# zuston/TonY

Hardware: AMD Instinct MI355X
Metric: images/sec (whole node) Inception-v3 TF-PS (higher is better)
Workload: dtype bf16

## Files before the change

### tony_amd/models/inception_v3.py

```python
from __future__ import annotations

import os

import torch
from torch import nn

from ..ops.concat import Slot, assemble, concat_buffer
from ..ops.dropout import Dropout as TonyDropout
from ..ops.pool import avg_pool, avg_pool3x3_s1, global_avg_pool, max_pool
from ..ops import conv as conv_ops
from ..ops import streams, tape
from ..ops.fused import FusedHead
from ..ops.residual import GradJoin
from ..ops.linear import Linear
from ..ops.x3 import ConvBNActX3, LinearX3, split_act
from .layers import ConvBNAct, conv_bn_act_maxpool, init_weights


JOIN = os.environ.get("TONY_INCEPTION_JOIN", "1") != "0"


def _join(t: torch.Tensor, n: int) -> None:
    if JOIN and t.is_cuda and t.dtype in (torch.bfloat16, torch.float32) and torch.is_grad_enabled() \
            and t.requires_grad:
        t._tony_join = GradJoin(n)


def _x3_input(x: torch.Tensor) -> None:
    if x.is_cuda and x.dtype == torch.float32:
        split_act(x)

# ... 365 lines not shown
            stem = (self.stem, self.stem2)
            segs = [(self._stem_fwd, [p for m in stem for p in m.parameters()], [b for m in stem for b in m.buffers()])]
            for blk in (*self.mixed_5, self.mixed_6a, *self.mixed_6):
                segs.append((blk, list(blk.parameters()), list(blk.buffers())))
            tail = [(blk, list(blk.parameters()), list(blk.buffers())) for blk in self.mixed_7]
            segs = self._tape_segs = (segs, tail)
        return segs

    def forward(self, x):
        if (self.fused and self.training and x.is_cuda and tape.ENABLED and torch.is_grad_enabled()
                and x.shape[0] * 64 >= conv_ops.MIN_ROWS):
            head, tail = self._segments()
            for run, params, bufs in head:
                x = tape.segment(run, x, params, bufs)
            aux = self.aux(x) if self.aux is not None else None
            for run, params, bufs in tail:
                x = tape.segment(run, x, params, bufs)
        else:
            x = self._stem_fwd(x)
            x = self.mixed_6(self.mixed_6a(self.mixed_5(x)))
            aux = self.aux(x) if (self.aux is not None and self.training) else None
            x = self.mixed_7(x)
        if self.fused or self.x3:
            x = global_avg_pool(x)
        else:
            x = torch.flatten(nn.functional.adaptive_avg_pool2d(x, 1), 1)
        logits = self.fc(self.dropout(x))
        return (logits, aux) if aux is not None else logits


def inception_v3(num_classes=1000, aux_logits=True, fused=True, seed=0, precision: str = "bf16") -> InceptionV3:
    if precision not in ("bf16", "fp32"):
        raise ValueError(f"precision must be bf16 or fp32, not {precision!r}")
    return init_weights(InceptionV3(num_classes, aux_logits, fused=fused, x3=precision == "fp32"), seed)
```

### tony_amd/models/resnet.py

```python
from __future__ import annotations

import os

import torch
from torch import nn

from ..ops import conv as conv_ops
from ..ops.bn import BatchNormAct2d
from ..ops.linear import Linear
from ..ops.pool import global_avg_pool
from ..ops.residual import GradJoin, bn_add_relu, conv1x1_bn_add_relu
from .layers import ConvBNAct, conv_bn_act_maxpool, init_weights


JOIN = os.environ.get("TONY_RESNET_JOIN", "1") != "0"
DS_TONY = os.environ.get("TONY_RESNET_DS_TONY", "1") != "0"


class Bottleneck(nn.Module):
    expansion = 4

    def __init__(self, cin, width, stride=1, fused=True, eps=1e-5):
        super().__init__()
        cout = width * self.expansion
        self.fused = fused
        self.conv1 = ConvBNAct(cin, width, 1, fused=fused, eps=eps)
        self.conv2 = ConvBNAct(width, width, 3, stride=stride, padding=1, fused=fused, eps=eps)
        self.conv3 = nn.Conv2d(width, cout, 1, bias=False)
        self.bn3 = nn.BatchNorm2d(cout, eps=eps)
        self.downsample = None
        if stride != 1 or cin != cout:
            self.downsample = nn.Sequential(
                nn.Conv2d(cin, cout, 1, stride=stride, bias=False),
# ... 26 lines not shown


class ResNet(nn.Module):
    def __init__(self, layers=(3, 4, 6, 3), num_classes=1000, fused=True, eps=1e-5):
        super().__init__()
        self.fused = fused
        self.stem = ConvBNAct(3, 64, 7, stride=2, padding=3, fused=fused, eps=eps)
        blocks = []
        cin = 64
        for i, n in enumerate(layers):
            width = 64 * 2 ** i
            for j in range(n):
                blocks.append(Bottleneck(cin, width, stride=2 if (j == 0 and i > 0) else 1, fused=fused, eps=eps))
                cin = width * Bottleneck.expansion
        self.blocks = nn.Sequential(*blocks)
        self.fc = (Linear if fused else nn.Linear)(cin, num_classes)

    def forward(self, x):
        if self.fused:
            x = conv_bn_act_maxpool(self.stem, x, 3, 2, padding=1)
        else:
            x = torch.nn.functional.max_pool2d(self.stem(x), 3, 2, 1)
        x = self.blocks(x)
        x = global_avg_pool(x) if self.fused else x.mean((2, 3))
        return self.fc(x)


def resnet50(num_classes: int = 1000, fused: bool = True, seed: int = 0) -> ResNet:
    m = ResNet((3, 4, 6, 3), num_classes, fused=fused)
    init_weights(m, seed)
    for b in m.blocks:
        nn.init.zeros_(b.bn3.weight)
    return m
```

### tony_amd/ops/_lib.py

```python
from __future__ import annotations

import ctypes
import os
import threading
import weakref
from typing import Dict

import torch

_HERE = os.path.dirname(os.path.abspath(__file__))
SO_PATH = os.environ.get("TONY_KERNELS_SO") or os.path.join(_HERE, "_tony_kernels.so")

_lock = threading.Lock()
_lib = None

c_void_p = ctypes.c_void_p
c_int = ctypes.c_int
c_int64 = ctypes.c_int64
c_float = ctypes.c_float
c_int_p = ctypes.POINTER(ctypes.c_int)
c_void_pp = ctypes.POINTER(ctypes.c_void_p)
c_u8_p = ctypes.POINTER(ctypes.c_uint8)
c_u64_p = ctypes.POINTER(ctypes.c_uint64)

# ... 50 lines not shown
    "tony_sgd_step": [c_void_p, c_void_p, c_void_p, c_int, c_void_p, c_int64, c_void_p, c_void_p],
    "tony_adam_step": [c_void_p, c_void_p, c_void_p, c_void_p, c_int, c_void_p, c_int64, c_void_p, c_void_p],
    "tony_adagrad_step": [c_void_p, c_void_p, c_void_p, c_int, c_void_p, c_int64, c_void_p, c_void_p],
    "tony_rmsprop_step": [c_void_p, c_void_p, c_void_p, c_void_p, c_int, c_void_p, c_int64, c_void_p, c_void_p],
    "tony_grad_stats": [c_void_p, c_int, c_int64, c_void_p, c_void_p],
    "tony_grad_sumsq_blocks": [],
    "tony_grad_sumsq": [c_void_p, c_int, c_int64, c_void_p, c_void_p],
    "tony_clip_ctl": [c_void_p, c_int, c_void_p, c_void_p, c_void_p],
    "tony_optim_apply_x": [c_int, c_void_p, c_void_p, c_void_p, c_void_p, c_void_p, c_int, c_void_p, c_int64,
                           c_void_p, c_void_p, c_void_p, c_void_p],
    "tony_layerwise_item_floats": [],
    "tony_lars_norm": [c_void_p, c_void_p, c_int, c_void_p, c_int64, c_void_p, c_int, c_void_p, c_void_p, c_void_p],
    "tony_lamb_norm": [c_void_p, c_void_p, c_void_p, c_void_p, c_int, c_int64, c_void_p, c_int, c_void_p, c_void_p,
                       c_void_p, c_void_p, c_void_p],
    "tony_layerwise_fold": [c_void_p, c_void_p, c_void_p, c_int, c_void_p, c_void_p],
    "tony_layerwise_ratio": [c_int, c_void_p, c_void_p, c_int, c_void_p, c_void_p, c_void_p, c_void_p],
    "tony_lars_apply": [c_void_p, c_void_p, c_void_p, c_void_p, c_int, c_void_p, c_int64, c_void_p, c_int, c_void_p,
                        c_void_p, c_void_p, c_void_p, c_void_p],
    "tony_lamb_apply": [c_void_p, c_void_p, c_void_p, c_void_p, c_void_p, c_int64, c_void_p, c_int, c_void_p,
                        c_void_p, c_void_p, c_void_p, c_void_p],
    "tony_xent_fwd": [c_void_p, c_int, c_int64, c_int, c_int64, c_void_p, c_float, c_void_p, c_void_p, c_void_p],
    "tony_xent_bwd": [c_void_p, c_int, c_int64, c_int, c_int64, c_void_p, c_float, c_void_p, c_void_p, c_void_p,
                      c_int64, c_void_p],
    "tony_image_preprocess": [c_void_p, c_int, c_void_p, c_void_p, c_int, c_int, c_int, c_int, c_int, c_int, c_float,
                              c_float, c_float, c_float, c_float, c_float, c_void_p],
    "tony_image_colour_scratch_floats": [c_int, c_int, c_int],
    "tony_image_preprocess_colour": [c_void_p, c_int, c_void_p, c_void_p, c_int, c_void_p, c_int64, c_void_p, c_int,
                                     c_int, c_int, c_int, c_int, c_int, c_float, c_float, c_float, c_float, c_float,
                                     c_float, c_void_p],
    "tony_topk_count": [c_void_p, c_int, c_int64, c_int, c_int64, c_void_p, c_int, c_void_p, c_void_p],
    "tony_dropout_fwd": [c_void_p, c_void_p, c_void_p, c_int64, c_int, c_float, c_void_p, c_void_p],
    "tony_dropout_bwd": [c_void_p, c_void_p, c_void_p, c_int64, c_int, c_float, c_void_p],
    "tony_counter_bump": [c_void_p, c_void_p],
    "tony_gemm_bf16": [c_void_p, c_void_p, c_void_p, c_int64, c_int64, c_int64, c_int64, c_int64, c_int64,
                       c_int, c_void_p, c_int64, c_void_p],
    "tony_gemm_bf16_bnact": [c_void_p, c_void_p, c_void_p, c_int64, c_int64, c_int64, c_int64, c_int64, c_int64,
                             c_int, c_void_p, c_int64, c_void_p, c_void_p],
    "tony_gemm_tn_bf16": [c_void_p, c_void_p, c_void_p, c_int64, c_int64, c_int64, c_int64, c_int64, c_int64,
                          c_void_p, c_int64, c_void_p, c_int, c_void_p, c_void_p, c_int, c_void_p],
    "tony_splitk_reduce": [c_void_p, c_int, c_int64, c_void_p, c_int, c_int, c_int, c_void_p],
    "tony_splitk_workspace": [c_void_p, c_int64, c_void_p, c_int64],
    "tony_conv_fwd": [c_void_p, c_int, c_int, c_int, c_int, c_int64, c_void_p, c_int, c_int, c_int, c_int, c_int,
                      c_int, c_int, c_void_p, c_int, c_int, c_int64, c_int, c_void_p, c_int64, c_void_p],
    "tony_stem_fwd": [c_void_p, c_int, c_int, c_int, c_int, c_void_p, c_int, c_int, c_int, c_int, c_int, c_int,
                      c_int, c_void_p, c_int, c_int, c_int64, c_int, c_void_p, c_int64, c_int, c_void_p],
    "tony_stem_wgrad": [c_void_p, c_int64, c_void_p, c_int, c_int, c_int, c_int, c_int, c_int, c_int, c_int, c_int,
# ... 371 lines not shown
```

### tony_amd/ops/conv.py

```python
from __future__ import annotations

import ctypes
import os
import weakref
from typing import Callable, Dict, Tuple

import torch

from . import _lib, concat, streams, tape, tune, wt_cache
from .arena import zeros_f32
from .bn import HOST_MEMO, _accum_ok, _as_rows, _rows_view
from .gemm import occ_choices, splitk_combine, wgrad_cus, wgrad_tn

_BF16 = torch.bfloat16
AUTOTUNE = os.environ.get("TONY_CONV_AUTOTUNE", "1") != "0"
_CHOICE: Dict[Tuple, str] = {}


def _pair(v):
    if type(v) is tuple:
        return v
    return tuple(v) if isinstance(v, (tuple, list)) else (int(v), int(v))


STEM = os.environ.get("TONY_STEM", "1") != "0"
MIN_ROWS = int(os.environ.get("TONY_CONV_MIN_ROWS", "1"))


_SUP_CACHE: dict = {}


def supported(x: torch.Tensor, weight: torch.Tensor, stride=1, padding=0, dilation=1, groups=1,
# ... 296 lines not shown
    return x if _rows_view(x)[2] == x.shape[1] else x.contiguous(memory_format=torch.channels_last)


def _gemm_fwd(x, weight, stats=None):
    x = _dense_rows(x)
    n = x.shape[0]
    co = weight.shape[0]
    k = x[0].numel()
    _lib.check_stat_buffer(stats, co)
    wk = _krsc(weight).reshape(co, k)
    y = _cl_empty(n, co, 1, 1, x.device)
    vf = tune.gemm_flags(x, wk, y, n, co, k, k, stats is not None, tune.SMALL_GEMM_VARIANTS)
    rc = _lib.lib().tony_gemm_bf16(x.data_ptr(), wk.data_ptr(), y.data_ptr(), n, co, k, k, k, co,
                                   (1 if stats is not None else 0) | vf, _lib.ptr(stats),
                                   2 * co if stats is not None else 0, _lib.stream_ptr(x.device))
    _lib.check(rc, "tony_gemm_bf16 (whole-input conv)")
    return y


def _gemm_dgrad(dy, weight, x_shape):
    dy, (_, co, lddy) = _as_rows(dy)
    n, c, h, w = x_shape
    k = c * h * w
    wt = _krsc(weight).reshape(co, k).t().contiguous()
    dx = _cl_empty(n, c, h, w, dy.device)
    if lddy != co:
        dy = dy.contiguous(memory_format=torch.channels_last)
        lddy = co
    vf = tune.gemm_flags(dy, wt, dx, n, k, co, lddy, False, tune.SMALL_GEMM_VARIANTS)
    rc = _lib.lib().tony_gemm_bf16(dy.data_ptr(), wt.data_ptr(), dx.data_ptr(), n, k, co, lddy, co, k, vf, 0, 0,
                                   _lib.stream_ptr(dy.device))
    _lib.check(rc, "tony_gemm_bf16 (whole-input conv dgrad)")
    return dx


def _gemm_wgrad(dy, x, weight_shape, dst=None):
    dy, (_, co, lddy) = _as_rows(dy)
    x = _dense_rows(x)
    n = x.shape[0]
    k = x[0].numel()
    if n % 8 == 0 and (dst is None or dst.dtype in (torch.float32, _BF16)):
        dev = x.device
        dyt = torch.as_strided(dy, (co, n), (1, lddy)).contiguous()
        xt = x.permute(0, 2, 3, 1).reshape(n, k).t().contiguous()
        out = dst if dst is not None else torch.empty(co * k, dtype=torch.float32, device=dev)
        base = (8 if out.dtype == torch.float32 else 0) | (16 if dst is not None else 0)
        scratch = torch.empty(co * k, dtype=_BF16, device=dev)
# ... 412 lines not shown
```

### tony_amd/ops/csrc/loss.hip

```cpp
#include "common.h"

using namespace tony;

namespace {

constexpr int kThreads = 256;
constexpr int kPerThread = 16;

template <bool kBf16>
__device__ __forceinline__ float ld(const void* p, int64_t i) {
  if constexpr (kBf16) return bf2f(static_cast<const uint16_t*>(p)[i]);
  return static_cast<const float*>(p)[i];
}

__device__ __forceinline__ float block_reduce(float v, float* sh, bool is_max) {
  v = is_max ? wave_max(v) : wave_sum(v);
  const int lane = threadIdx.x & (kWave - 1), wid = threadIdx.x / kWave;
  __syncthreads();
  if (lane == 0) sh[wid] = v;
  __syncthreads();
  float r = sh[0];
#pragma unroll
  for (int k = 1; k < kThreads / kWave; ++k) r = is_max ? fmaxf(r, sh[k]) : r + sh[k];
  return r;
}

template <bool kBf16>
__global__ __launch_bounds__(kThreads) void xent_fwd_kernel(const void* __restrict__ logits, int64_t ld_,
                                                            int K, const int64_t* __restrict__ labels,
                                                            float smoothing, float* __restrict__ loss,
                                                            float* __restrict__ lse_out) {
  __shared__ float sh[kThreads / kWave];
  const int64_t row = blockIdx.x;
  const int64_t base = row * ld_;
  float v[kPerThread];
  float mx = -INFINITY;
#pragma unroll
  for (int j = 0; j < kPerThread; ++j) {
    const int k = threadIdx.x + j * kThreads;
    v[j] = k < K ? ld<kBf16>(logits, base + k) : -INFINITY;
    mx = fmaxf(mx, v[j]);
  }
  mx = block_reduce(mx, sh, true);
  float se = 0.f, sx = 0.f;
#pragma unroll
  for (int j = 0; j < kPerThread; ++j) {
    const int k = threadIdx.x + j * kThreads;
    if (k < K) {
      se += __expf(v[j] - mx);
      sx += v[j];
    }
  }
  se = block_reduce(se, sh, false);
  sx = block_reduce(sx, sh, false);
  if (threadIdx.x == 0) {
    const float lse = mx + __logf(se);
    const int64_t t = labels[row];
    const bool live = t >= 0 && t < K;
    const float xt = live ? ld<kBf16>(logits, base + t) : lse;
    float l = (1.f - smoothing) * (lse - xt);
    if (smoothing != 0.f) l += smoothing * (lse - sx / static_cast<float>(K));
    loss[row] = live ? l : 0.f;
    lse_out[row] = lse;
  }
}

template <bool kBf16>
__global__ __launch_bounds__(kThreads) void xent_bwd_kernel(const void* __restrict__ logits, int64_t ld_,
                                                            int K, const int64_t* __restrict__ labels,
                                                            float smoothing, const float* __restrict__ lse,
                                                            const float* __restrict__ gout,
                                                            void* __restrict__ dlogits, int64_t ldd) {
  const int64_t row = blockIdx.x;
  const float l = lse[row];
  const float go = gout[row];
  const int64_t t = labels[row];
  const bool live = t >= 0 && t < K;
  const float off = smoothing / static_cast<float>(K);
  for (int k = threadIdx.x; k < K; k += kThreads) {
    const float p = __expf(ld<kBf16>(logits, row * ld_ + k) - l);
    const float target = (k == t ? 1.f - smoothing : 0.f) + off;
    const float d = live ? (p - target) * go : 0.f;
    if constexpr (kBf16)
      static_cast<uint16_t*>(dlogits)[row * ldd + k] = f2bf(d);
    else
      static_cast<float*>(dlogits)[row * ldd + k] = d;
  }
}

}

TONY_API int tony_xent_fwd(const void* logits, int is_bf16, int64_t N, int K, int64_t ld_,
                           const int64_t* labels, float smoothing, float* loss, float* lse,
                           hipStream_t stream) {
  if (K <= 0 || K > kThreads * kPerThread) return -1;
  if (N <= 0) return 0;
  if (is_bf16)
    xent_fwd_kernel<true><<<N, kThreads, 0, stream>>>(logits, ld_, K, labels, smoothing, loss, lse);
  else
    xent_fwd_kernel<false><<<N, kThreads, 0, stream>>>(logits, ld_, K, labels, smoothing, loss, lse);
  TONY_LAUNCH_CHECK();
  return 0;
}

TONY_API int tony_xent_bwd(const void* logits, int is_bf16, int64_t N, int K, int64_t ld_,
                           const int64_t* labels, float smoothing, const float* lse, const float* gout,
                           void* dlogits, int64_t ldd, hipStream_t stream) {
  if (K <= 0) return -1;
  if (N <= 0) return 0;
  if (is_bf16)
    xent_bwd_kernel<true><<<N, kThreads, 0, stream>>>(logits, ld_, K, labels, smoothing, lse, gout, dlogits, ldd);
  else
    xent_bwd_kernel<false><<<N, kThreads, 0, stream>>>(logits, ld_, K, labels, smoothing, lse, gout, dlogits, ldd);
  TONY_LAUNCH_CHECK();
  return 0;
}
```

### tony_amd/ops/linear.py

```python
from __future__ import annotations

import os

import torch
from torch import nn

from . import _lib, tape, tune
from .gemm import wgrad_tn

_BF16 = torch.bfloat16
TUNE = os.environ.get("TONY_LINEAR_TUNE", "1") != "0"


def supported(x: torch.Tensor, weight: torch.Tensor) -> bool:
    return (x.is_cuda and x.dtype == _BF16 and weight.dtype == _BF16 and x.dim() == 2
            and weight.shape[1] % 8 == 0 and weight.shape[0] % 8 == 0 and x.shape[1] == weight.shape[1])


def _affine(bias: torch.Tensor | None, n: int, device) -> torch.Tensor:
    aff = torch.zeros(2 * n, dtype=torch.float32, device=device)
    aff[:n] = 1.0
    if bias is not None:
        aff[n:] = bias.float()
    return aff


class _LinearFn(torch.autograd.Function):
    @staticmethod
    def forward(ctx, x, weight, bias):
        L = _lib.lib()
        if x.stride(1) != 1 or x.data_ptr() % 16 or x.stride(0) % 8:
            x = x.contiguous()
        w = weight if weight.is_contiguous() else weight.contiguous()
        m, k = x.shape
        n = w.shape[0]
        y = torch.empty((m, n), dtype=x.dtype, device=x.device)
        aff = _affine(bias, n, x.device)
        vf = tune.gemm_flags(x, w, y, m, n, k, x.stride(0), False) if TUNE else 0
        rc = L.tony_gemm_bf16(x.data_ptr(), w.data_ptr(), y.data_ptr(), m, n, k, x.stride(0), k, n, 2 | vf,
                              aff.data_ptr(), 0, _lib.stream_ptr(x.device))
        _lib.check(rc, "tony_gemm_bf16 (linear)")
        ctx.save_for_backward(x, w)
        ctx.has_bias = bias is not None
        ctx.params = (weight, bias)
        return y

    @staticmethod
    def backward(ctx, dy):
        x, w = ctx.saved_tensors
        weight, bias = ctx.params
        L, dev = _lib.lib(), x.device
        st = _lib.stream_ptr(dev)
        if dy.stride(1) != 1 or dy.data_ptr() % 16 or dy.stride(0) % 8:
            dy = dy.contiguous()
        m, k = x.shape
        n = w.shape[0]
        dx = dw = db = None
        if ctx.needs_input_grad[0]:
            wt = w.t().contiguous()
            dx = torch.empty((m, k), dtype=x.dtype, device=dev)
            vf = tune.gemm_flags(dy, wt, dx, m, k, n, dy.stride(0), False) if TUNE else 0
            rc = L.tony_gemm_bf16(dy.data_ptr(), wt.data_ptr(), dx.data_ptr(), m, k, n, dy.stride(0), n, k, vf, 0, 0,
                                  st)
            _lib.check(rc, "tony_gemm_bf16 (linear dgrad)")
        if ctx.needs_input_grad[1]:
            gw = _lib.grad_slot(weight)
            if gw is not None and gw.is_contiguous():
                wgrad_tn(dy.data_ptr(), dy.stride(0), x.data_ptr(), x.stride(0), m, n, k, dev, dst=gw)
            else:
                dw = wgrad_tn(dy.data_ptr(), dy.stride(0), x.data_ptr(), x.stride(0), m, n, k, dev).to(weight.dtype)
        if ctx.has_bias and ctx.needs_input_grad[2]:
            db = dy.float().sum(0)
            gb = _lib.grad_slot(bias)
            if gb is not None:
                gb.add_(db.to(gb.dtype))
                db = None
            else:
                db = db.to(bias.dtype)
        _lib.report_inplace((weight, bias), (dw, db))
        return dx, dw, db


def linear(x: torch.Tensor, weight: torch.Tensor, bias: torch.Tensor | None = None) -> torch.Tensor:
    if supported(x, weight):
        return tape.apply(_LinearFn, x, weight, bias)
    return nn.functional.linear(x, weight, bias)


class Linear(nn.Linear):

    def forward(self, x):
        return linear(x, self.weight, self.bias)
```

### tony_amd/ops/loss.py

```python
from __future__ import annotations

import torch

from . import _lib


class _XentFn(torch.autograd.Function):
    @staticmethod
    def forward(ctx, logits, labels, smoothing):
        L = _lib.lib()
        if logits.stride(1) != 1:
            logits = logits.contiguous()
        labels = labels.contiguous().to(torch.int64)
        n, k = logits.shape
        is_bf16 = int(logits.dtype == torch.bfloat16)
        if not is_bf16 and logits.dtype != torch.float32:
            raise TypeError(f"cross_entropy kernel takes bf16/fp32 logits, got {logits.dtype}")
        loss = torch.empty(n, dtype=torch.float32, device=logits.device)
        lse = torch.empty(n, dtype=torch.float32, device=logits.device)
        rc = L.tony_xent_fwd(logits.data_ptr(), is_bf16, n, k, logits.stride(0), labels.data_ptr(), float(smoothing),
                             loss.data_ptr(), lse.data_ptr(), _lib.stream_ptr(logits.device))
        _lib.check(rc, "tony_xent_fwd")
        ctx.save_for_backward(logits, labels, lse)
        ctx.smoothing = smoothing
        return loss

    @staticmethod
    def backward(ctx, gout):
        L = _lib.lib()
        logits, labels, lse = ctx.saved_tensors
        n, k = logits.shape
        gout = gout.float().contiguous()
        if gout.numel() != n:
            gout = gout.expand(n).contiguous()
        d = torch.empty((n, k), dtype=logits.dtype, device=logits.device)
        rc = L.tony_xent_bwd(logits.data_ptr(), int(logits.dtype == torch.bfloat16), n, k, logits.stride(0),
                             labels.data_ptr(), float(ctx.smoothing), lse.data_ptr(), gout.data_ptr(), d.data_ptr(), k,
                             _lib.stream_ptr(logits.device))
        _lib.check(rc, "tony_xent_bwd")
        return d, None, None


def cross_entropy(logits: torch.Tensor, labels: torch.Tensor, label_smoothing: float = 0.0,
                  reduction: str = "mean") -> torch.Tensor:
    if logits.is_cuda:
        per_row = _XentFn.apply(logits, labels, label_smoothing)
    else:
        valid = (labels >= 0) & (labels < logits.shape[1])
        per_row = torch.nn.functional.cross_entropy(logits.float(), torch.where(valid, labels, -100),
                                                    reduction="none", ignore_index=-100,
                                                    label_smoothing=label_smoothing)
    if reduction == "mean":
        return per_row.mean()
    if reduction == "sum":
        return per_row.sum()
    return per_row
```

### tony_amd/ops/pool.py

```python
from __future__ import annotations

import torch

from . import _lib, concat, streams, tape
from .bn import _as_rows, _rows_view


def _nhwc_empty(n, c, h, w, like):
    return torch.empty((n, c, h, w), dtype=like.dtype, device=like.device, memory_format=torch.channels_last)


def _fn(name: str, t: torch.Tensor):
    return getattr(_lib.lib(), name + "_f32" if t.dtype == torch.float32 else name)


def _ok(x: torch.Tensor) -> bool:
    return x.is_cuda and x.dtype in (torch.bfloat16, torch.float32) and x.shape[1] % 8 == 0


def _dense_rows(t: torch.Tensor, shape) -> bool:
    if tuple(t.shape) != tuple(shape) or t.data_ptr() % 16:
        return False
    rv = _rows_view(t)
    return rv is not None and rv[2] == t.shape[1]


def _box3(src, n, c, h, w, ld_src):
# ... 98 lines not shown
        _lib.check(rc, "tony_avgpool_fwd")
        ctx.shape = (n, c, h, w, k, s)
        return y

    @staticmethod
    def backward(ctx, dy):
        n, c, h, w, k, s = ctx.shape
        dy, (_, _, lddy) = _as_rows(dy)
        dx = _nhwc_empty(n, c, h, w, dy)
        rc = _fn("tony_avgpool_bwd", dy)(dy.data_ptr(), dx.data_ptr(), n, h, w, c, k, s, lddy, c,
                                         _lib.stream_ptr(dy.device))
        _lib.check(rc, "tony_avgpool_bwd")
        return dx, None, None


def avg_pool(x: torch.Tensor, k: int, s: int) -> torch.Tensor:
    if _ok(x):
        return tape.apply(_AvgPoolFn, x, k, s)
    return torch.nn.functional.avg_pool2d(x, k, s)


def global_avg_pool(x: torch.Tensor) -> torch.Tensor:
    if x.shape[2] == x.shape[3]:
        return torch.flatten(avg_pool(x, x.shape[2], 1), 1)
    return torch.flatten(torch.nn.functional.adaptive_avg_pool2d(x, 1), 1)


def avg_pool3x3_s1(x: torch.Tensor, planes_only: bool = False) -> torch.Tensor:
    if _ok(x):
        planes_only = planes_only and x.dtype == torch.float32 and not tape.recording()
        _LAST_PLANES[0] = None
        y = tape.apply(_AvgPool3Fn, x, planes_only)
        planes = _LAST_PLANES[0]
        if planes is not None:
            _LAST_PLANES[0] = None
            y._tony_x3 = (y._version, planes, x.shape[1])
        return y
    return torch.nn.functional.avg_pool2d(x, 3, 1, 1, count_include_pad=True)


def max_pool(x: torch.Tensor, k: int = 3, s: int = 2, slot=None, padding: int = 0) -> torch.Tensor:
    if _ok(x) and 2 * padding <= k:
        return tape.apply(_MaxPoolFn, x, k, s, slot, padding)
    return torch.nn.functional.max_pool2d(x, k, s, padding)
```

### tony_amd/ops/wt_cache.py

```python
from __future__ import annotations

import struct
from typing import Dict, Optional

import torch

from . import _lib

_DESC = struct.Struct("<QQiiiiii")
_T = 64


def _crsk(weight: torch.Tensor) -> torch.Tensor:
    return weight.permute(1, 2, 3, 0).contiguous()


class TransposedWeights:
    def __init__(self, device):
        self.device = _norm(device)
        if _lib.lib().tony_transpose_desc_bytes() != _DESC.size:
            raise _lib.KernelError("transpose descriptor layout differs between Python and the kernels")
        self.entries: Dict[int, tuple] = {}
        self.enabled = False
        self.frozen = False
        self.desc: Optional[torch.Tensor] = None
        self.n_desc = 0
        self.total_tiles = 0

    def get(self, weight: torch.Tensor) -> Optional[torch.Tensor]:
        if not self.enabled or not isinstance(weight, torch.nn.Parameter) or weight.dim() != 4:
            return None
        e = self.entries.get(id(weight))
        if e is not None and e[0] is weight and e[2] == weight.data_ptr():
            return e[1]
        if self.frozen or torch.cuda.is_current_stream_capturing():
            return None
        co, ci, r, s = weight.shape
        if not weight.is_contiguous(memory_format=torch.channels_last) or weight.dtype != torch.bfloat16:
            return None
        buf = _crsk(weight)
        self.entries[id(weight)] = (weight, buf, weight.data_ptr())
        self._build()
        return buf

    def _build(self):
        parts, tiles = [], 0
        for w, buf, _ in self.entries.values():
            co, ci, r, s = w.shape
            tci, tco = (ci + _T - 1) // _T, (co + _T - 1) // _T
            parts.append(_DESC.pack(w.data_ptr(), buf.data_ptr(), co, r * s, ci, tci, tco, tiles))
            tiles += r * s * tci * tco
        raw = torch.frombuffer(bytearray(b"".join(parts)), dtype=torch.uint8)
        self.desc = raw.to(self.device)
        self.n_desc = len(parts)
        self.total_tiles = tiles

    def refresh(self) -> None:
        if not self.n_desc:
            return
        L = _lib.lib()
        rc = L.tony_transpose_batch(self.desc.data_ptr(), self.n_desc, self.total_tiles,
                                    _lib.stream_ptr(self.device))
        _lib.check(rc, "tony_transpose_batch")


_XDESC = struct.Struct("<QQQiiiiiiii")


class X3Weights:

    def __init__(self, device):
        self.device = _norm(device)
        if _lib.lib().tony_x3_desc_bytes() != _XDESC.size:
            raise _lib.KernelError("x3 weight descriptor layout differs between Python and the kernels")
# ... 63 lines not shown
        d = torch.device("cuda", torch.cuda.current_device())
    return d


def activate(cache: Optional[TransposedWeights], x3cache: Optional[X3Weights] = None) -> None:
    _ACTIVE[0] = cache
    _ACTIVE_X3[0] = x3cache


def x3_planes(weight: torch.Tensor) -> Optional[torch.Tensor]:
    c = _ACTIVE_X3[0]
    if c is not None and c.enabled and c.device == _norm(weight.device):
        return c.planes(weight)
    return None


def x3_planes_t(weight: torch.Tensor) -> Optional[torch.Tensor]:
    c = _ACTIVE_X3[0]
    if c is not None and c.enabled and c.device == _norm(weight.device):
        return c.planes_t(weight)
    return None


def transposed(weight: torch.Tensor) -> torch.Tensor:
    c = _ACTIVE[0]
    if c is not None and c.enabled and c.device == _norm(weight.device):
        t = c.get(weight)
        if t is not None:
            return t
    return _crsk(weight)
```

Before: 9752.

## Fuse classifier head: pool+dropout kernel, mean-xent, cached flat weight transposes, bias colsum

Adds HIP kernels that fuse global average pooling with dropout in forward and backward, and a cross-entropy kernel that folds the batch mean in-kernel using a last-block counter. The fc bias gradient is accumulated directly into the grad slot, and flat transposed weights for the fc and flat conv backward are cached in the batched transpose cache. The goal is to cut the many small launches and copies in the classifier head and loss. In exchange it adds a new dropout RNG path and atomic counter state that must work under graph capture.

```diff
diff --git a/tony_amd/models/inception_v3.py b/tony_amd/models/inception_v3.py
--- a/tony_amd/models/inception_v3.py
+++ b/tony_amd/models/inception_v3.py
@@ -7,6 +7,7 @@
 
 from ..ops.concat import Slot, assemble, concat_buffer
 from ..ops.dropout import Dropout as TonyDropout
+from ..ops.head import pool_dropout
 from ..ops.pool import avg_pool, avg_pool3x3_s1, global_avg_pool, max_pool
 from ..ops import conv as conv_ops
 from ..ops import streams, tape
@@ -418,10 +419,10 @@
             aux = self.aux(x) if (self.aux is not None and self.training) else None
             x = self.mixed_7(x)
         if self.fused or self.x3:
-            x = global_avg_pool(x)
-        else:
-            x = torch.flatten(nn.functional.adaptive_avg_pool2d(x, 1), 1)
-        logits = self.fc(self.dropout(x))
+            x = pool_dropout(x, self.dropout)
+        else:
+            x = self.dropout(torch.flatten(nn.functional.adaptive_avg_pool2d(x, 1), 1))
+        logits = self.fc(x)
         return (logits, aux) if aux is not None else logits
 
 
diff --git a/tony_amd/models/resnet.py b/tony_amd/models/resnet.py
--- a/tony_amd/models/resnet.py
+++ b/tony_amd/models/resnet.py
@@ -8,7 +8,7 @@
 from ..ops import conv as conv_ops
 from ..ops.bn import BatchNormAct2d
 from ..ops.linear import Linear
-from ..ops.pool import global_avg_pool
+from ..ops.head import pool_dropout
 from ..ops.residual import GradJoin, bn_add_relu, conv1x1_bn_add_relu
 from .layers import ConvBNAct, conv_bn_act_maxpool, init_weights
 
@@ -81,7 +81,7 @@
         else:
             x = torch.nn.functional.max_pool2d(self.stem(x), 3, 2, 1)
         x = self.blocks(x)
-        x = global_avg_pool(x) if self.fused else x.mean((2, 3))
+        x = pool_dropout(x) if self.fused else x.mean((2, 3))
         return self.fc(x)
 
 
diff --git a/tony_amd/ops/_lib.py b/tony_amd/ops/_lib.py
--- a/tony_amd/ops/_lib.py
+++ b/tony_amd/ops/_lib.py
@@ -96,6 +96,16 @@
     "tony_xent_fwd": [c_void_p, c_int, c_int64, c_int, c_int64, c_void_p, c_float, c_void_p, c_void_p, c_void_p],
     "tony_xent_bwd": [c_void_p, c_int, c_int64, c_int, c_int64, c_void_p, c_float, c_void_p, c_void_p, c_void_p,
                       c_int64, c_void_p],
+    "tony_xent_fwd_mean": [c_void_p, c_int, c_int64, c_int, c_int64, c_void_p, c_float, c_void_p, c_void_p, c_void_p,
+                           c_void_p, c_void_p],
+    "tony_xent_bwd_mean": [c_void_p, c_int, c_int64, c_int, c_int64, c_void_p, c_float, c_void_p, c_void_p, c_void_p,
+                           c_int64, c_void_p],
+    "tony_head_pool_dropout_fwd": [c_void_p, c_void_p, c_void_p, c_int, c_int, c_int, c_int64, c_int64, c_float,
+                                   c_void_p, c_void_p],
+    "tony_head_pool_dropout_bwd": [c_void_p, c_void_p, c_void_p, c_int, c_int, c_int, c_int64, c_int64, c_float,
+                                   c_void_p],
+    "tony_head_affine": [c_void_p, c_int, c_int, c_void_p, c_void_p],
+    "tony_colsum_accum": [c_void_p, c_int64, c_int, c_int, c_void_p, c_int, c_void_p],
     "tony_image_preprocess": [c_void_p, c_int, c_void_p, c_void_p, c_int, c_int, c_int, c_int, c_int, c_int, c_float,
                               c_float, c_float, c_float, c_float, c_float, c_void_p],
     "tony_image_colour_scratch_floats": [c_int, c_int, c_int],
diff --git a/tony_amd/ops/conv.py b/tony_amd/ops/conv.py
--- a/tony_amd/ops/conv.py
+++ b/tony_amd/ops/conv.py
@@ -7,7 +7,7 @@
 
 import torch
 
-from . import _lib, concat, streams, tape, tune, wt_cache
+from . import _lib, concat, head, streams, tape, tune, wt_cache
 from .arena import zeros_f32
 from .bn import HOST_MEMO, _accum_ok, _as_rows, _rows_view
 from .gemm import occ_choices, splitk_combine, wgrad_cus, wgrad_tn
@@ -350,7 +350,7 @@
     dy, (_, co, lddy) = _as_rows(dy)
     n, c, h, w = x_shape
     k = c * h * w
-    wt = _krsc(weight).reshape(co, k).t().contiguous()
+    wt = wt_cache.transposed_flat(weight) if head.FUSED else _krsc(weight).reshape(co, k).t().contiguous()
     dx = _cl_empty(n, c, h, w, dy.device)
     if lddy != co:
         dy = dy.contiguous(memory_format=torch.channels_last)
diff --git a/tony_amd/ops/csrc/head.hip b/tony_amd/ops/csrc/head.hip
--- /dev/null
+++ b/tony_amd/ops/csrc/head.hip
@@ -0,0 +1,193 @@
+#include "common.h"
+
+using namespace tony;
+
+namespace {
+
+constexpr int kLanes = 64;
+constexpr int kThreads = 256;
+
+__device__ __forceinline__ uint64_t mix64(uint64_t z) {
+  z += 0x9e3779b97f4a7c15ull;
+  z = (z ^ (z >> 30)) * 0xbf58476d1ce4e5b9ull;
+  z = (z ^ (z >> 27)) * 0x94d049bb133111ebull;
+  return z ^ (z >> 31);
+}
+
+__device__ __forceinline__ unsigned keep_bits(const int64_t* rng, int64_t g, uint32_t thr) {
+  const uint64_t key =
+      mix64(static_cast<uint64_t>(rng[0]) ^ mix64(static_cast<uint64_t>(rng[1]) + 0x632be59bd9b4e019ull));
+  const uint64_t h0 = mix64(key + 2 * static_cast<uint64_t>(g)), h1 = mix64(key + 2 * static_cast<uint64_t>(g) + 1);
+  unsigned bits = 0;
+#pragma unroll
+  for (int e = 0; e < 8; ++e) {
+    const uint32_t r = static_cast<uint32_t>(((e < 4 ? h0 : h1) >> (16 * (e & 3))) & 0xffffu);
+    bits |= (r >= thr ? 1u : 0u) << e;
+  }
+  return bits;
+}
+
+__global__ __launch_bounds__(kLanes) void head_pool_dropout_fwd_kernel(
+    const uint16_t* __restrict__ x, uint16_t* __restrict__ y, uint8_t* __restrict__ mask, int HW, int CG, int groups,
+    int64_t ldx, int64_t ldy, float inv, uint32_t thr, float scale, const int64_t* __restrict__ rng) {
+  const int64_t n = blockIdx.x / groups;
+  const int cg = (blockIdx.x % groups) * kLanes + threadIdx.x;
+  if (cg >= CG) return;
+  const uint16_t* p = x + n * HW * ldx + cg * 8;
+  float acc[8] = {0, 0, 0, 0, 0, 0, 0, 0};
+  int s = 0;
+  for (; s + 8 <= HW; s += 8) {
+    bf16x8 v[8];
+#pragma unroll
+    for (int u = 0; u < 8; ++u) v[u] = load8(p + (s + u) * ldx);
+#pragma unroll
+    for (int u = 0; u < 8; ++u) {
+      float f[8];
+      v[u].to_float(f);
+#pragma unroll
+      for (int j = 0; j < 8; ++j) acc[j] += f[j];
+    }
+  }
+  for (; s < HW; ++s) {
+    float f[8];
+    load8(p + s * ldx).to_float(f);
+#pragma unroll
+    for (int j = 0; j < 8; ++j) acc[j] += f[j];
+  }
+#pragma unroll
+  for (int j = 0; j < 8; ++j) acc[j] *= inv;
+  bf16x8 out = bf16x8::from_float(acc);
+  if (mask != nullptr) {
+    const int64_t g = n * CG + cg;
+    const unsigned bits = keep_bits(rng, g, thr);
+    mask[g] = static_cast<uint8_t>(bits);
+    out.to_float(acc);
+#pragma unroll
+    for (int j = 0; j < 8; ++j) acc[j] = ((bits >> j) & 1u) ? acc[j] * scale : 0.f;
+    out = bf16x8::from_float(acc);
+  }
+  store8(y + n * ldy + cg * 8, out);
+}
+
+__global__ __launch_bounds__(kThreads) void head_pool_dropout_bwd_kernel(
+    const uint16_t* __restrict__ dy, uint16_t* __restrict__ dx, const uint8_t* __restrict__ mask, int HW, int CG,
+    int64_t total, int64_t lddy, int64_t lddx, float inv, float scale) {
+  const int64_t t = static_cast<int64_t>(blockIdx.x) * kThreads + threadIdx.x;
+  if (t >= total) return;
+  const int cg = static_cast<int>(t % CG);
+  const int64_t site = t / CG;
+  const int64_t n = site / HW;
+  float g[8];
+  load8(dy + n * lddy + cg * 8).to_float(g);
+  if (mask != nullptr) {
+    const unsigned bits = mask[n * CG + cg];
+#pragma unroll
+    for (int j = 0; j < 8; ++j) g[j] = ((bits >> j) & 1u) ? g[j] * scale : 0.f;
+    bf16x8::from_float(g).to_float(g);
+  }
+#pragma unroll
+  for (int j = 0; j < 8; ++j) g[j] = (0.f + g[j]) * inv;
+  store8(dx + site * lddx + cg * 8, bf16x8::from_float(g));
+}
+
+__global__ __launch_bounds__(kThreads) void head_affine_kernel(const void* __restrict__ bias, int is_bf16, int n,
+                                                               float* __restrict__ aff) {
+  const int i = blockIdx.x * kThreads + threadIdx.x;
+  if (i >= n) return;
+  aff[i] = 1.f;
+  aff[n + i] = bias == nullptr ? 0.f
+               : is_bf16      ? bf2f(static_cast<const uint16_t*>(bias)[i])
+                              : static_cast<const float*>(bias)[i];
+}
+
+template <bool kSlotBf16>
+__global__ __launch_bounds__(kLanes) void colsum_accum_kernel(const uint16_t* __restrict__ dy, int64_t ld, int M,
+                                                              int N, void* __restrict__ slot) {
+  const int c0 = (blockIdx.x * kLanes + threadIdx.x) * 8;
+  if (c0 >= N) return;
+  float acc[8] = {0, 0, 0, 0, 0, 0, 0, 0};
+  const uint16_t* p = dy + c0;
+  int m = 0;
+  for (; m + 8 <= M; m += 8) {
+    bf16x8 v[8];
+#pragma unroll
+    for (int u = 0; u < 8; ++u) v[u] = load8(p + (m + u) * ld);
+#pragma unroll
+    for (int u = 0; u < 8; ++u) {
+      float f[8];
+      v[u].to_float(f);
+#pragma unroll
+      for (int j = 0; j < 8; ++j) acc[j] += f[j];
+    }
+  }
+  for (; m < M; ++m) {
+    float f[8];
+    load8(p + m * ld).to_float(f);
+#pragma unroll
+    for (int j = 0; j < 8; ++j) acc[j] += f[j];
+  }
+#pragma unroll
+  for (int j = 0; j < 8; ++j) {
+    if constexpr (kSlotBf16) {
+      uint16_t* s = static_cast<uint16_t*>(slot) + c0 + j;
+      *s = f2bf(bf2f(*s) + acc[j]);
+    } else {
+      float* s = static_cast<float*>(slot) + c0 + j;
+      *s += acc[j];
+    }
+  }
+}
+
+}
+
+TONY_API int tony_head_pool_dropout_fwd(const void* x, void* y, void* mask, int N, int HW, int C, int64_t ldx,
+                                        int64_t ldy, float p, const int64_t* rng, hipStream_t stream) {
+  if (N <= 0) return 0;
+  if (HW <= 0 || C <= 0 || C % 8 || ldx % 8 || ldy % 8 || ldx < C || ldy < C) return -1;
+  if (mask != nullptr && (!(p >= 0.f && p < 1.f) || rng == nullptr)) return -1;
+  if ((reinterpret_cast<uintptr_t>(x) | reinterpret_cast<uintptr_t>(y)) & 15) return -3;
+  const int CG = C / 8, groups = ceil_div(CG, kLanes);
+  if (static_cast<int64_t>(N) * groups > 0x7fffffff) return -1;
+  const uint32_t thr = static_cast<uint32_t>(p * 65536.f + 0.5f);
+  head_pool_dropout_fwd_kernel<<<N * groups, kLanes, 0, stream>>>(
+      static_cast<const uint16_t*>(x), static_cast<uint16_t*>(y), static_cast<uint8_t*>(mask), HW, CG, groups, ldx,
+      ldy, 1.f / static_cast<float>(HW), thr, 1.f / (1.f - p), rng);
+  TONY_LAUNCH_CHECK();
+  return 0;
+}
+
+TONY_API int tony_head_pool_dropout_bwd(const void* dy, void* dx, const void* mask, int N, int HW, int C,
+                                        int64_t lddy, int64_t lddx, float p, hipStream_t stream) {
+  if (N <= 0) return 0;
+  if (HW <= 0 || C <= 0 || C % 8 || lddy % 8 || lddx % 8 || lddy < C || lddx < C) return -1;
+  if (mask != nullptr && !(p >= 0.f && p < 1.f)) return -1;
+  if ((reinterpret_cast<uintptr_t>(dy) | reinterpret_cast<uintptr_t>(dx)) & 15) return -3;
+  const int64_t total = static_cast<int64_t>(N) * HW * (C / 8);
+  if (total > 0x7fffffffll * kThreads) return -1;
+  head_pool_dropout_bwd_kernel<<<ceil_div(total, kThreads), kThreads, 0, stream>>>(
+      static_cast<const uint16_t*>(dy), static_cast<uint16_t*>(dx), static_cast<const uint8_t*>(mask), HW, C / 8,
+      total, lddy, lddx, 1.f / static_cast<float>(HW), 1.f / (1.f - p));
+  TONY_LAUNCH_CHECK();
+  return 0;
+}
+
+TONY_API int tony_head_affine(const void* bias, int is_bf16, int n, float* aff, hipStream_t stream) {
+  if (n <= 0 || aff == nullptr) return -1;
+  head_affine_kernel<<<ceil_div(n, kThreads), kThreads, 0, stream>>>(bias, is_bf16, n, aff);
+  TONY_LAUNCH_CHECK();
+  return 0;
+}
+
+TONY_API int tony_colsum_accum(const void* dy, int64_t ld, int M, int N, void* slot, int slot_is_bf16,
+                               hipStream_t stream) {
+  if (M < 0 || N <= 0 || N % 8 || ld % 8 || ld < N || slot == nullptr) return -1;
+  if (reinterpret_cast<uintptr_t>(dy) & 15) return -3;
+  if (M == 0) return 0;
+  const int blocks = ceil_div(N / 8, kLanes);
+  if (slot_is_bf16)
+    colsum_accum_kernel<true><<<blocks, kLanes, 0, stream>>>(static_cast<const uint16_t*>(dy), ld, M, N, slot);
+  else
+    colsum_accum_kernel<false><<<blocks, kLanes, 0, stream>>>(static_cast<const uint16_t*>(dy), ld, M, N, slot);
+  TONY_LAUNCH_CHECK();
+  return 0;
+}
diff --git a/tony_amd/ops/csrc/loss.hip b/tony_amd/ops/csrc/loss.hip
--- a/tony_amd/ops/csrc/loss.hip
+++ b/tony_amd/ops/csrc/loss.hip
@@ -26,10 +26,9 @@
 }
 
 template <bool kBf16>
-__global__ __launch_bounds__(kThreads) void xent_fwd_kernel(const void* __restrict__ logits, int64_t ld_,
-                                                            int K, const int64_t* __restrict__ labels,
-                                                            float smoothing, float* __restrict__ loss,
-                                                            float* __restrict__ lse_out) {
+__device__ __forceinline__ void xent_fwd_row(const void* __restrict__ logits, int64_t ld_, int K,
+                                             const int64_t* __restrict__ labels, float smoothing, float* loss,
+                                             float* __restrict__ lse_out) {
   __shared__ float sh[kThreads / kWave];
   const int64_t row = blockIdx.x;
   const int64_t base = row * ld_;
@@ -66,14 +65,55 @@
 }
 
 template <bool kBf16>
+__global__ __launch_bounds__(kThreads) void xent_fwd_kernel(const void* __restrict__ logits, int64_t ld_,
+                                                            int K, const int64_t* __restrict__ labels,
+                                                            float smoothing, float* __restrict__ loss,
+                                                            float* __restrict__ lse_out) {
+  xent_fwd_row<kBf16>(logits, ld_, K, labels, smoothing, loss, lse_out);
+}
+
+__device__ __forceinline__ void xent_mean_fold(float* loss, int N, unsigned* counter, float* mean) {
+  __shared__ double part[kThreads];
+  __shared__ int s_last;
+  if (threadIdx.x == 0) {
+    __threadfence();
+    s_last = atomicAdd(counter, 1u) == static_cast<unsigned>(N - 1);
+  }
+  __syncthreads();
+  if (!s_last) return;
+  __builtin_amdgcn_fence(__ATOMIC_ACQUIRE, "agent");
+  const int per = (N + kThreads - 1) / kThreads;
+  double s = 0.0;
+  for (int r = threadIdx.x * per; r < min(N, (static_cast<int>(threadIdx.x) + 1) * per); ++r)
+    s += static_cast<double>(__hip_atomic_load(loss + r, __ATOMIC_RELAXED, __HIP_MEMORY_SCOPE_AGENT));
+  part[threadIdx.x] = s;
+  __syncthreads();
+  if (threadIdx.x == 0) {
+    double t = 0.0;
+    for (int k = 0; k < kThreads; ++k) t += part[k];
+    *mean = static_cast<float>(t / static_cast<double>(N));
+    __hip_atomic_store(counter, 0u, __ATOMIC_RELAXED, __HIP_MEMORY_SCOPE_AGENT);
+  }
+}
+
+template <bool kBf16>
+__global__ __launch_bounds__(kThreads) void xent_fwd_mean_kernel(const void* __restrict__ logits, int64_t ld_, int K,
+                                                                 const int64_t* __restrict__ labels, float smoothing,
+                                                                 float* loss, float* __restrict__ lse_out, int N,
+                                                                 unsigned* counter, float* mean) {
+  xent_fwd_row<kBf16>(logits, ld_, K, labels, smoothing, loss, lse_out);
+  xent_mean_fold(loss, N, counter, mean);
+}
+
+template <bool kBf16, bool kMean>
 __global__ __launch_bounds__(kThreads) void xent_bwd_kernel(const void* __restrict__ logits, int64_t ld_,
                                                             int K, const int64_t* __restrict__ labels,
                                                             float smoothing, const float* __restrict__ lse,
-                                                            const float* __restrict__ gout,
+                                                            const float* __restrict__ gout, float inv_n,
                                                             void* __restrict__ dlogits, int64_t ldd) {
   const int64_t row = blockIdx.x;
   const float l = lse[row];
-  const float go = gout[row];
+  const float go = kMean ? gout[0] * inv_n : gout[row];
   const int64_t t = labels[row];
   const bool live = t >= 0 && t < K;
   const float off = smoothing / static_cast<float>(K);
@@ -109,9 +149,42 @@
   if (K <= 0) return -1;
   if (N <= 0) return 0;
   if (is_bf16)
-    xent_bwd_kernel<true><<<N, kThreads, 0, stream>>>(logits, ld_, K, labels, smoothing, lse, gout, dlogits, ldd);
+    xent_bwd_kernel<true, false><<<N, kThreads, 0, stream>>>(logits, ld_, K, labels, smoothing, lse, gout, 0.f,
+                                                             dlogits, ldd);
   else
-    xent_bwd_kernel<false><<<N, kThreads, 0, stream>>>(logits, ld_, K, labels, smoothing, lse, gout, dlogits, ldd);
+    xent_bwd_kernel<false, false><<<N, kThreads, 0, stream>>>(logits, ld_, K, labels, smoothing, lse, gout, 0.f,
+                                                              dlogits, ldd);
   TONY_LAUNCH_CHECK();
   return 0;
 }
+
+TONY_API int tony_xent_fwd_mean(const void* logits, int is_bf16, int64_t N, int K, int64_t ld_,
+                                const int64_t* labels, float smoothing, float* loss, float* lse, float* mean,
+                                unsigned* counter, hipStream_t stream) {
+  if (K <= 0 || K > kThreads * kPerThread || N <= 0 || N > (1 << 20) || mean == nullptr || counter == nullptr)
+    return -1;
+  const int n = static_cast<int>(N);
+  if (is_bf16)
+    xent_fwd_mean_kernel<true><<<n, kThreads, 0, stream>>>(logits, ld_, K, labels, smoothing, loss, lse, n, counter,
+                                                           mean);
+  else
+    xent_fwd_mean_kernel<false><<<n, kThreads, 0, stream>>>(logits, ld_, K, labels, smoothing, loss, lse, n, counter,
+                                                            mean);
+  TONY_LAUNCH_CHECK();
+  return 0;
+}
+
+TONY_API int tony_xent_bwd_mean(const void* logits, int is_bf16, int64_t N, int K, int64_t ld_,
+                                const int64_t* labels, float smoothing, const float* lse, const float* gout,
+                                void* dlogits, int64_t ldd, hipStream_t stream) {
+  if (K <= 0 || N <= 0 || gout == nullptr) return -1;
+  const float inv_n = 1.f / static_cast<float>(N);
+  if (is_bf16)
+    xent_bwd_kernel<true, true><<<N, kThreads, 0, stream>>>(logits, ld_, K, labels, smoothing, lse, gout, inv_n,
+                                                            dlogits, ldd);
+  else
+    xent_bwd_kernel<false, true><<<N, kThreads, 0, stream>>>(logits, ld_, K, labels, smoothing, lse, gout, inv_n,
+                                                             dlogits, ldd);
+  TONY_LAUNCH_CHECK();
+  return 0;
+}
diff --git a/tony_amd/ops/head.py b/tony_amd/ops/head.py
--- /dev/null
+++ b/tony_amd/ops/head.py
@@ -0,0 +1,93 @@
+from __future__ import annotations
+
+import os
+
+import torch
+
+from . import _lib, tape
+from .bn import _as_rows
+
+FUSED = os.environ.get("TONY_FUSED_HEAD", "1") != "0"
+_BF16 = torch.bfloat16
+
+
+def _rows2d(t: torch.Tensor) -> torch.Tensor:
+    if t.stride(1) != 1 or t.data_ptr() % 16 or (t.shape[0] > 1 and (t.stride(0) % 8 or t.stride(0) < t.shape[1])):
+        t = t.contiguous()
+    return t
+
+
+class _PoolDropoutFn(torch.autograd.Function):
+    @staticmethod
+    def forward(ctx, x, p, rng):
+        x, (_, c, ld) = _as_rows(x)
+        n, _, h, w = x.shape
+        L, st = _lib.lib(), _lib.stream_ptr(x.device)
+        y = torch.empty((n, c), dtype=x.dtype, device=x.device)
+        mask = None
+        if p > 0.0:
+            if rng.device != x.device or rng.dtype != torch.int64 or rng.numel() != 2:
+                raise ValueError("dropout rng state must be an int64 [seed, counter] tensor on the input's device")
+            mask = torch.empty(n * c // 8, dtype=torch.uint8, device=x.device)
+        _lib.check(L.tony_head_pool_dropout_fwd(x.data_ptr(), y.data_ptr(), _lib.ptr(mask), n, h * w, c, ld, c,
+                                                float(p), _lib.ptr(rng) if mask is not None else 0, st),
+                   "tony_head_pool_dropout_fwd")
+        if mask is not None:
+            _lib.check(L.tony_counter_bump(rng.data_ptr(), st), "tony_counter_bump")
+            ctx.save_for_backward(mask)
+        ctx.p = p
+        ctx.shape = (n, c, h, w)
+        return y
+
+    @staticmethod
+    def backward(ctx, gy):
+        n, c, h, w = ctx.shape
+        mask = ctx.saved_tensors[0] if ctx.p > 0.0 else None
+        gy = _rows2d(gy)
+        dx = torch.empty((n, c, h, w), dtype=gy.dtype, device=gy.device, memory_format=torch.channels_last)
+        _lib.check(_lib.lib().tony_head_pool_dropout_bwd(gy.data_ptr(), dx.data_ptr(), _lib.ptr(mask), n, h * w, c,
+                                                         gy.stride(0) if n > 1 else c, c, float(ctx.p),
+                                                         _lib.stream_ptr(gy.device)),
+                   "tony_head_pool_dropout_bwd")
+        return dx, None, None
+
+
+def fused_pool_ok(x: torch.Tensor) -> bool:
+    return (FUSED and x.is_cuda and x.dtype == _BF16 and x.dim() == 4 and x.shape[1] % 8 == 0
+            and x.shape[2] == x.shape[3] and x.shape[0] > 0)
+
+
+def pool_dropout(x: torch.Tensor, drop=None) -> torch.Tensor:
+    from .pool import global_avg_pool
+
+    p = drop.p if drop is not None and drop.training else 0.0
+    if not fused_pool_ok(x) or x.shape[2] == 1 or (p > 0.0 and not hasattr(drop, "rng")):
+        y = global_avg_pool(x)
+        return y if drop is None else drop(y)
+    return tape.apply(_PoolDropoutFn, x, p, drop.rng if p > 0.0 else None)
+
+
+def bias_affine(bias, n: int, device) -> torch.Tensor:
+    aff = torch.empty(2 * n, dtype=torch.float32, device=device)
+    if bias is not None and not bias.is_contiguous():
+        bias = bias.contiguous()
+    rc = _lib.lib().tony_head_affine(_lib.ptr(bias), int(bias is not None and bias.dtype == _BF16), n,
+                                     aff.data_ptr(), _lib.stream_ptr(device))
+    _lib.check(rc, "tony_head_affine")
+    return aff
+
+
+def affine_ok(bias) -> bool:
+    return FUSED and (bias is None or bias.dtype in (_BF16, torch.float32))
+
+
+def colsum_accum(dy: torch.Tensor, slot: torch.Tensor) -> bool:
+    m, n = dy.shape
+    if not (FUSED and dy.is_cuda and dy.dtype == _BF16 and n % 8 == 0 and slot.dtype in (_BF16, torch.float32)
+            and slot.dim() == 1 and slot.numel() == n and slot.stride(0) == 1):
+        return False
+    dy = _rows2d(dy)
+    rc = _lib.lib().tony_colsum_accum(dy.data_ptr(), dy.stride(0) if m > 1 else n, m, n, slot.data_ptr(),
+                                      int(slot.dtype == _BF16), _lib.stream_ptr(dy.device))
+    _lib.check(rc, "tony_colsum_accum")
+    return True
diff --git a/tony_amd/ops/linear.py b/tony_amd/ops/linear.py
--- a/tony_amd/ops/linear.py
+++ b/tony_amd/ops/linear.py
@@ -5,7 +5,7 @@
 import torch
 from torch import nn
 
-from . import _lib, tape, tune
+from . import _lib, head, tape, tune, wt_cache
 from .gemm import wgrad_tn
 
 _BF16 = torch.bfloat16
@@ -35,7 +35,7 @@
         m, k = x.shape
         n = w.shape[0]
         y = torch.empty((m, n), dtype=x.dtype, device=x.device)
-        aff = _affine(bias, n, x.device)
+        aff = head.bias_affine(bias, n, x.device) if head.affine_ok(bias) else _affine(bias, n, x.device)
         vf = tune.gemm_flags(x, w, y, m, n, k, x.stride(0), False) if TUNE else 0
         rc = L.tony_gemm_bf16(x.data_ptr(), w.data_ptr(), y.data_ptr(), m, n, k, x.stride(0), k, n, 2 | vf,
                               aff.data_ptr(), 0, _lib.stream_ptr(x.device))
@@ -57,7 +57,7 @@
         n = w.shape[0]
         dx = dw = db = None
         if ctx.needs_input_grad[0]:
-            wt = w.t().contiguous()
+            wt = wt_cache.transposed_flat(weight) if head.FUSED and weight.is_contiguous() else w.t().contiguous()
             dx = torch.empty((m, k), dtype=x.dtype, device=dev)
             vf = tune.gemm_flags(dy, wt, dx, m, k, n, dy.stride(0), False) if TUNE else 0
             rc = L.tony_gemm_bf16(dy.data_ptr(), wt.data_ptr(), dx.data_ptr(), m, k, n, dy.stride(0), n, k, vf, 0, 0,
@@ -70,13 +70,14 @@
             else:
                 dw = wgrad_tn(dy.data_ptr(), dy.stride(0), x.data_ptr(), x.stride(0), m, n, k, dev).to(weight.dtype)
         if ctx.has_bias and ctx.needs_input_grad[2]:
-            db = dy.float().sum(0)
             gb = _lib.grad_slot(bias)
-            if gb is not None:
-                gb.add_(db.to(gb.dtype))
-                db = None
-            else:
-                db = db.to(bias.dtype)
+            if gb is None or not head.colsum_accum(dy, gb):
+                db = dy.float().sum(0)
+                if gb is not None:
+                    gb.add_(db.to(gb.dtype))
+                    db = None
+                else:
+                    db = db.to(bias.dtype)
         _lib.report_inplace((weight, bias), (dw, db))
         return dx, dw, db
 
diff --git a/tony_amd/ops/loss.py b/tony_amd/ops/loss.py
--- a/tony_amd/ops/loss.py
+++ b/tony_amd/ops/loss.py
@@ -2,7 +2,7 @@
 
 import torch
 
-from . import _lib
+from . import _lib, head
 
 
 class _XentFn(torch.autograd.Function):
@@ -41,9 +41,68 @@
         return d, None, None
 
 
+_COUNTERS: dict = {}
+_N_COUNTERS = 64
+
+
+def _counter(device) -> int:
+    idx = device.index if device.index is not None else torch.cuda.current_device()
+    c = _COUNTERS.get(idx)
+    if c is None:
+        if torch.cuda.is_current_stream_capturing():
+            return 0
+        c = _COUNTERS[idx] = [torch.zeros(_N_COUNTERS, dtype=torch.int32, device=device), 0]
+    c[1] = (c[1] + 1) % _N_COUNTERS
+    return c[0].data_ptr() + 4 * c[1]
+
+
+class _XentMeanFn(torch.autograd.Function):
+
+    @staticmethod
+    def forward(ctx, logits, labels, smoothing, counter):
+        L = _lib.lib()
+        if logits.stride(1) != 1:
+            logits = logits.contiguous()
+        labels = labels.contiguous().to(torch.int64)
+        n, k = logits.shape
+        loss = torch.empty(n, dtype=torch.float32, device=logits.device)
+        lse = torch.empty(n, dtype=torch.float32, device=logits.device)
+        mean = torch.empty((), dtype=torch.float32, device=logits.device)
+        rc = L.tony_xent_fwd_mean(logits.data_ptr(), int(logits.dtype == torch.bfloat16), n, k, logits.stride(0),
+                                  labels.data_ptr(), float(smoothing), loss.data_ptr(), lse.data_ptr(),
+                                  mean.data_ptr(), counter, _lib.stream_ptr(logits.device))
+        _lib.check(rc, "tony_xent_fwd_mean")
+        ctx.save_for_backward(logits, labels, lse)
+        ctx.smoothing = smoothing
+        ctx.mark_non_differentiable(loss, lse)
+        return mean, loss, lse
+
+    @staticmethod
+    def backward(ctx, gout, _gloss, _glse):
+        logits, labels, lse = ctx.saved_tensors
+        n, k = logits.shape
+        if gout.dtype != torch.float32 or gout.numel() != 1:
+            raise TypeError("the mean loss takes one fp32 gradient")
+        d = torch.empty((n, k), dtype=logits.dtype, device=logits.device)
+        rc = _lib.lib().tony_xent_bwd_mean(logits.data_ptr(), int(logits.dtype == torch.bfloat16), n, k,
+                                           logits.stride(0), labels.data_ptr(), float(ctx.smoothing), lse.data_ptr(),
+                                           gout.data_ptr(), d.data_ptr(), k, _lib.stream_ptr(logits.device))
+        _lib.check(rc, "tony_xent_bwd_mean")
+        return d, None, None, None
+
+
+def _mean_ok(logits: torch.Tensor) -> bool:
+    return (head.FUSED and logits.dim() == 2 and logits.dtype in (torch.bfloat16, torch.float32)
+            and 0 < logits.shape[0] <= 1 << 20 and 0 < logits.shape[1] <= 4096)
+
+
 def cross_entropy(logits: torch.Tensor, labels: torch.Tensor, label_smoothing: float = 0.0,
                   reduction: str = "mean") -> torch.Tensor:
     if logits.is_cuda:
+        if reduction == "mean" and _mean_ok(logits):
+            counter = _counter(logits.device)
+            if counter:
+                return _XentMeanFn.apply(logits, labels, label_smoothing, counter)[0]
         per_row = _XentFn.apply(logits, labels, label_smoothing)
     else:
         valid = (labels >= 0) & (labels < logits.shape[1])
diff --git a/tony_amd/ops/pool.py b/tony_amd/ops/pool.py
--- a/tony_amd/ops/pool.py
+++ b/tony_amd/ops/pool.py
@@ -2,7 +2,7 @@
 
 import torch
 
-from . import _lib, concat, streams, tape
+from . import _lib, concat, head, streams, tape
 from .bn import _as_rows, _rows_view
 
 
@@ -147,6 +147,8 @@
 
 def global_avg_pool(x: torch.Tensor) -> torch.Tensor:
     if x.shape[2] == x.shape[3]:
+        if x.shape[2] == 1 and head.FUSED and x.is_cuda and x.dtype == torch.bfloat16:
+            return torch.flatten(x, 1)
         return torch.flatten(avg_pool(x, x.shape[2], 1), 1)
     return torch.flatten(torch.nn.functional.adaptive_avg_pool2d(x, 1), 1)
 
diff --git a/tony_amd/ops/wt_cache.py b/tony_amd/ops/wt_cache.py
--- a/tony_amd/ops/wt_cache.py
+++ b/tony_amd/ops/wt_cache.py
@@ -13,6 +13,11 @@
 
 def _crsk(weight: torch.Tensor) -> torch.Tensor:
     return weight.permute(1, 2, 3, 0).contiguous()
+
+
+def _kc(weight: torch.Tensor) -> torch.Tensor:
+    w = weight if weight.dim() == 2 else weight.permute(0, 2, 3, 1).reshape(weight.shape[0], -1)
+    return w.t().contiguous()
 
 
 class TransposedWeights:
@@ -21,6 +26,7 @@
         if _lib.lib().tony_transpose_desc_bytes() != _DESC.size:
             raise _lib.KernelError("transpose descriptor layout differs between Python and the kernels")
         self.entries: Dict[int, tuple] = {}
+        self.flat: Dict[int, tuple] = {}
         self.enabled = False
         self.frozen = False
         self.desc: Optional[torch.Tensor] = None
@@ -43,13 +49,30 @@
         self._build()
         return buf
 
+    def get_flat(self, weight: torch.Tensor) -> Optional[torch.Tensor]:
+        if not self.enabled or not isinstance(weight, torch.nn.Parameter) or weight.dim() not in (2, 4):
+            return None
+        e = self.flat.get(id(weight))
+        if e is not None and e[0] is weight and e[2] == weight.data_ptr():
+            return e[1]
+        if self.frozen or torch.cuda.is_current_stream_capturing():
+            return None
+        fmt = torch.contiguous_format if weight.dim() == 2 else torch.channels_last
+        if not weight.is_contiguous(memory_format=fmt) or weight.dtype != torch.bfloat16:
+            return None
+        buf = _kc(weight)
+        self.flat[id(weight)] = (weight, buf, weight.data_ptr())
+        self._build()
+        return buf
+
     def _build(self):
         parts, tiles = [], 0
-        for w, buf, _ in self.entries.values():
-            co, ci, r, s = w.shape
+        shapes = [(w, buf, w.shape[0], w.shape[2] * w.shape[3], w.shape[1]) for w, buf, _ in self.entries.values()]
+        shapes += [(w, buf, w.shape[0], 1, w[0].numel()) for w, buf, _ in self.flat.values()]
+        for w, buf, co, rs, ci in shapes:
             tci, tco = (ci + _T - 1) // _T, (co + _T - 1) // _T
-            parts.append(_DESC.pack(w.data_ptr(), buf.data_ptr(), co, r * s, ci, tci, tco, tiles))
-            tiles += r * s * tci * tco
+            parts.append(_DESC.pack(w.data_ptr(), buf.data_ptr(), co, rs, ci, tci, tco, tiles))
+            tiles += rs * tci * tco
         raw = torch.frombuffer(bytearray(b"".join(parts)), dtype=torch.uint8)
         self.desc = raw.to(self.device)
         self.n_desc = len(parts)
@@ -159,6 +182,15 @@
     return None
 
 
+def transposed_flat(weight: torch.Tensor) -> torch.Tensor:
+    c = _ACTIVE[0]
+    if c is not None and c.enabled and c.device == _norm(weight.device):
+        t = c.get_flat(weight)
+        if t is not None:
+            return t
+    return _kc(weight)
+
+
 def transposed(weight: torch.Tensor) -> torch.Tensor:
     c = _ACTIVE[0]
     if c is not None and c.enabled and c.device == _norm(weight.device):
```

New measurement: 9593. -1.6%, worse.
